# crockwell/far

Hardware: AMD Instinct MI355X
Metric: image-pairs/sec (match+solve+regress) at 640x480 (higher is better)
Workload: dtype f32

## Files before the change

far_amd/csrc/dual_softmax_f16s.hip:

```cpp
#include "k1_f16s.h"
#include <algorithm>

int far_k1_conf_launch(const _Float16* ah, const _Float16* bh, int Z, int L, int S, int Lp, int Sp, float c1, float fill2,
                       const uint8_t* mask0, const uint8_t* mask1, const float2* rowstat, const float* cmax,
                       const float* cinv, float* conf, const int* fix_count, const uint2* fix_list, int slots,
                       int* fix_info_out, hipStream_t stream);

namespace {

constexpr int CAND_SLOTS = 4;

#define FAR_DPP(old, v, ctrl, rowmask) \
    __builtin_bit_cast(float, __builtin_amdgcn_update_dpp(__builtin_bit_cast(int, old), __builtin_bit_cast(int, v), ctrl, rowmask, 0xF, false))
__device__ __forceinline__ float max32_to_upper_row(float v) {
    v = fmaxf(v, FAR_DPP(v, v, 0xB1, 0xF));
    v = fmaxf(v, FAR_DPP(v, v, 0x4E, 0xF));
    v = fmaxf(v, FAR_DPP(v, v, 0x141, 0xF));
    v = fmaxf(v, FAR_DPP(v, v, 0x140, 0xF));
    v = fmaxf(v, FAR_DPP(v, v, 0x142, 0xA));
    return v;
}

template <bool CAND>
__global__ __launch_bounds__(256, 2) void k1_rowstats(const _Float16* __restrict__ ah, const _Float16* __restrict__ al,
                                                      const _Float16* __restrict__ bh, const _Float16* __restrict__ bl,
                                                      int Z, int Nr, int Nc, int Nrp, int Ncp, float c1, float fill2,
                                                      const uint8_t* __restrict__ rmask, const uint8_t* __restrict__ cmask,
                                                      float2* __restrict__ stat, float* __restrict__ dmax, float* __restrict__ dinv,
                                                      float* __restrict__ dthr, const float* __restrict__ othr,
                                                      int* __restrict__ cand_count, uint2* __restrict__ cand) {
    extern __shared__ __attribute__((aligned(16))) unsigned char lds[];
    const int tid = threadIdx.x, wave = tid >> 6, lane = tid & 63, l31 = lane & 31, h = lane >> 5;
    int z, Ib;
    tile_coords(Nrp / 128, Z, z, Ib);
    const int irow = Ib * 128 + 32 * wave + l31;
    RowFrags rf;
    rf.load(ah, al, (size_t)z * Nrp + irow, irow, h);
    const bool rmasked = rmask && irow < Nr && !rmask[(size_t)z * Nr + irow];
    float m = -HUGE_F, sum = 0.f, comp = 0.f;
    int ncand = 0;
    const int ntile = (Nc + KT - 1) / KT;
    for (int jt = 0; jt < ntile; ++jt) {
        __syncthreads();
        dma_tile(lds, bh, bl, (size_t)z * Ncp + jt * KT, tid, wave);
        if (CAND && tid < KT)
            reinterpret_cast<float*>(lds + 2 * TILE_PLANE)[tid] = othr[(size_t)z * Ncp + jt * KT + tid];
        asm volatile("s_waitcnt vmcnt(0)" ::: "memory");
        __syncthreads();
        f32x16 acc[2];
        score_tile(acc, lds, rf, l31, h);
        const bool special = (jt + 1) * KT > Nc || cmask != nullptr || rmask != nullptr;
        float tm = -HUGE_F;
#pragma unroll
        for (int ct = 0; ct < 2; ++ct)
#pragma unroll
            for (int r = 0; r < 16; ++r) {
                float x = acc[ct][r] * c1;
                if (special) {
                    const int j = jt * KT + 32 * ct + mfma32_row(r, h);
                    if (j >= Nc) x = -HUGE_F;
                    else if (rmasked || (cmask && !cmask[(size_t)z * Nc + j])) x = fill2;
                }
                acc[ct][r] = x;
                tm = fmaxf(tm, x);
            }
        const float mn = fmaxf(m, tm);
        const float resc = __builtin_amdgcn_exp2f(m - mn);
        float t = 0.f;
#pragma unroll
        for (int ct = 0; ct < 2; ++ct)
#pragma unroll
            for (int r = 0; r < 16; ++r) t += __builtin_amdgcn_exp2f(acc[ct][r] - mn);
        sum *= resc;
        comp *= resc;
        const float y = t - comp;
        const float ns = sum + y;
        comp = (ns - sum) - y;
        sum = ns;
        m = mn;
        if (CAND) {
            const float clog = m + __builtin_amdgcn_logf(sum - comp);
            float hot = -1.f;
            const float* tl = reinterpret_cast<const float*>(lds + 2 * TILE_PLANE);
#pragma unroll
            for (int ct = 0; ct < 2; ++ct)
#pragma unroll
                for (int q4 = 0; q4 < 4; ++q4) {
                    const float4 a = *reinterpret_cast<const float4*>(tl + 32 * ct + 8 * q4 + 4 * h);
                    hot = fmaxf(hot, fmaxf(fmaxf(2.0f * acc[ct][4 * q4 + 0] - a.x, 2.0f * acc[ct][4 * q4 + 1] - a.y),
                                           fmaxf(2.0f * acc[ct][4 * q4 + 2] - a.z, 2.0f * acc[ct][4 * q4 + 3] - a.w)));
                }
            if (__builtin_amdgcn_ballot_w64(hot >= clog) != 0ull) {
                uint2* const slots = cand + ((size_t)z * Nr + min(irow, Nr - 1)) * (2 * CAND_SLOTS) + h * CAND_SLOTS;
#pragma unroll 1
                for (int ct = 0; ct < 2; ++ct)
#pragma unroll
                    for (int r = 0; r < 16; ++r) {
                        const int i = jt * KT + 32 * ct + mfma32_row(r, h);
                        const float xv = ct == 0 ? acc[0][r] : acc[1][r];
                        if (2.0f * xv >= tl[32 * ct + mfma32_row(r, h)] + clog && xv > -1.0e8f && i < Nc && irow < Nr) {
                            if (ncand < CAND_SLOTS) slots[ncand] = make_uint2((unsigned)i, __float_as_uint(xv));
                            ++ncand;
                        }
                    }
            }
        }
    }
    if (CAND && irow < Nr) cand_count[((size_t)z * Nr + irow) * 2 + h] = ncand;
    sum -= comp;
    const float mo = shfl_xor_f(m, 32), so = shfl_xor_f(sum, 32);
    const float mn = fmaxf(m, mo);
    const float st = sum * __builtin_amdgcn_exp2f(m - mn) + so * __builtin_amdgcn_exp2f(mo - mn);
    if (h == 0) {
        if (irow < Nr) stat[(size_t)z * Nr + irow] = make_float2(mn, st);
        if (dmax) {
            dmax[(size_t)z * Nrp + irow] = irow < Nr ? mn : HUGE_F;
            dinv[(size_t)z * Nrp + irow] = irow < Nr ? 1.0f / st : 0.f;
        }
        if (dthr) dthr[(size_t)z * Nrp + irow] = irow < Nr ? mn + __builtin_amdgcn_logf(st) - 12.0f : HUGE_F;
    }
}

__global__ __launch_bounds__(256, 2) void k1_screen(const _Float16* __restrict__ ah, const _Float16* __restrict__ bh, int Z, int L, int S,
                                                    int Lp, int Sp, float c1, const float2* __restrict__ rowstat,
                                                    const float* __restrict__ cmax, float thr, const unsigned* __restrict__ nmax,
                                                    uint8_t* __restrict__ tmask) {
    extern __shared__ __attribute__((aligned(16))) unsigned char lds[];
    const int tid = threadIdx.x, wave = tid >> 6, lane = tid & 63, l31 = lane & 31, h = lane >> 5;
    const int nI = Lp / 128;
    int z, Ib;
    tile_coords(nI, Z, z, Ib);
    const int irow = Ib * 128 + 32 * wave + l31;
    f16x8 rh[NS];
#pragma unroll
    for (int s = 0; s < NS; ++s)
        rh[s] = *reinterpret_cast<const f16x8*>(ah + ((size_t)z * Lp + irow) * C + 8 * ((2 * s + h) ^ (irow & 15)));
    const float rmax = irow < L ? rowstat[(size_t)z * L + irow].x : HUGE_F;
    const float c2 = 2.0f * c1;
    const float slack2 = c2 * __builtin_sqrtf(__uint_as_float(nmax[0]) * __uint_as_float(nmax[1])) *
                         (1.0f / 1024.0f * (1.0f + 1.0f / 2048.0f) + 1.0f / 8192.0f);
    const float lim = __builtin_amdgcn_logf(thr) + rmax - slack2;
    const int ntile = (S + KT - 1) / KT;
    for (int jt = 0; jt < ntile; ++jt) {
        __syncthreads();
        {
            const unsigned char* sh = reinterpret_cast<const unsigned char*>(bh + ((size_t)z * Sp + jt * KT) * C) + tid * 16;
#pragma unroll
            for (int j = 0; j < TILE_PLANE / 4096; ++j)
                __builtin_amdgcn_global_load_lds((gptr_t)(sh + j * 4096), (lptr_t)(lds + j * 4096 + wave * 1024), 16, 0, 0);
        }
        asm volatile("s_waitcnt vmcnt(0)" ::: "memory");
        __syncthreads();
        f32x16 acc[2];
#pragma unroll
        for (int ct = 0; ct < 2; ++ct)
#pragma unroll
            for (int r = 0; r < 16; ++r) acc[ct][r] = 0.f;
#pragma unroll
        for (int s = 0; s < NS; ++s)
#pragma unroll
            for (int ct = 0; ct < 2; ++ct) {
                const int row = 32 * ct + l31;
                const f16x8 ch = *reinterpret_cast<const f16x8*>(lds + row * ROWB + (((2 * s + h) ^ (row & 15)) * 16));
                acc[ct] = __builtin_amdgcn_mfma_f32_32x32x16_f16(ch, rh[s], acc[ct], 0, 0, 0);
            }
        float top = -HUGE_F;
#pragma unroll
        for (int ct = 0; ct < 2; ++ct)
#pragma unroll
            for (int q4 = 0; q4 < 4; ++q4) {
                const float4 a = *reinterpret_cast<const float4*>(cmax + (size_t)z * Sp + jt * KT + 32 * ct + 8 * q4 + 4 * h);
                top = fmaxf(top, fmaxf(fmaxf(fmaf(acc[ct][4 * q4 + 0], c2, -a.x), fmaf(acc[ct][4 * q4 + 1], c2, -a.y)),
                                       fmaxf(fmaf(acc[ct][4 * q4 + 2], c2, -a.z), fmaf(acc[ct][4 * q4 + 3], c2, -a.w))));
            }
        const bool can = !(top <= lim);
        const bool any = __builtin_amdgcn_ballot_w64(can) != 0ull;
        if (lane == 0) tmask[(((size_t)z * nI + Ib) * ntile + jt) * 4 + wave] = any ? 1 : 0;
    }
}

template <bool CONF>
__global__ __launch_bounds__(256, 2) void k1_match(const _Float16* __restrict__ ah, const _Float16* __restrict__ al,
                                                   const _Float16* __restrict__ bh, const _Float16* __restrict__ bl,
                                                   int Z, int L, int S, int Lp, int Sp, float c1, float fill2,
                                                   const uint8_t* __restrict__ mask0, const uint8_t* __restrict__ mask1,
                                                   const float2* __restrict__ rowstat, const float* __restrict__ cmax,
                                                   const float* __restrict__ cinv, float* __restrict__ conf,
                                                   float* __restrict__ rowbest_v, int* __restrict__ rowbest_j,
                                                   unsigned* __restrict__ colbest, float thr, const uint8_t* __restrict__ tmask) {
    extern __shared__ __attribute__((aligned(16))) unsigned char lds[];
    const int tid = threadIdx.x, wave = tid >> 6, lane = tid & 63, l31 = lane & 31, h = lane >> 5;
    const int nI = Lp / 128;
    int z, Ib;
    tile_coords(nI, Z, z, Ib);
    const int irow = Ib * 128 + 32 * wave + l31;
    const bool ivalid = irow < L;
    RowFrags rf;
    rf.load(ah, al, (size_t)z * Lp + irow, irow, h);
    const float2 rst = ivalid ? rowstat[(size_t)z * L + irow] : make_float2(0.f, 1.f);
    const float rinv = 1.0f / rst.y;
    const float c2 = 2.0f * c1;
    const bool rmasked = mask0 && ivalid && !mask0[(size_t)z * L + irow];
    const bool aligned4 = (S & 3) == 0;
    float bestv = -1.f;
    int bestj = 0x7fffffff;
    const int ntile = (S + KT - 1) / KT;
    for (int jt = 0; jt < ntile; ++jt) {
        if (tmask && *reinterpret_cast<const unsigned*>(tmask + (((size_t)z * nI + Ib) * ntile + jt) * 4) == 0u) continue;
        __syncthreads();
        dma_tile(lds, bh, bl, (size_t)z * Sp + jt * KT, tid, wave);
        asm volatile("s_waitcnt vmcnt(0)" ::: "memory");
        __syncthreads();
        if (tmask && tmask[(((size_t)z * nI + Ib) * ntile + jt) * 4 + wave] == 0) continue;
        f32x16 acc[2];
        score_tile(acc, lds, rf, l31, h);
        const bool masks = mask0 != nullptr || mask1 != nullptr;
#pragma unroll
        for (int ct = 0; ct < 2; ++ct) {
            float cm[16], ci[16];
#pragma unroll
            for (int q4 = 0; q4 < 4; ++q4) {
                const size_t o = (size_t)z * Sp + jt * KT + 32 * ct + 8 * q4 + 4 * h;
                const float4 a = *reinterpret_cast<const float4*>(cmax + o), b = *reinterpret_cast<const float4*>(cinv + o);
                cm[4 * q4 + 0] = a.x; cm[4 * q4 + 1] = a.y; cm[4 * q4 + 2] = a.z; cm[4 * q4 + 3] = a.w;
                ci[4 * q4 + 0] = b.x; ci[4 * q4 + 1] = b.y; ci[4 * q4 + 2] = b.z; ci[4 * q4 + 3] = b.w;
            }
#pragma unroll
            for (int r = 0; r < 16; ++r) {
                const int j = jt * KT + 32 * ct + mfma32_row(r, h);
                float x2 = acc[ct][r] * c2;
                if (masks && j < S && (rmasked || (mask1 && !mask1[(size_t)z * S + j]))) x2 = 2.0f * fill2;
                const float p = __builtin_amdgcn_exp2f((x2 - rst.x) - cm[r]) * rinv * ci[r];
                const bool valid = ivalid && j < S;
                acc[ct][r] = valid ? p : -1.f;
                if (valid && p > bestv) { bestv = p; bestj = j; }
            }
            if (CONF && ivalid) {
#pragma unroll
                for (int q4 = 0; q4 < 4; ++q4) {
                    const int j = jt * KT + 32 * ct + 8 * q4 + 4 * h;
                    float* dst = conf + ((size_t)z * L + irow) * S + j;
                    if (aligned4 && j + 3 < S) {
                        *reinterpret_cast<float4*>(dst) = make_float4(acc[ct][4 * q4], acc[ct][4 * q4 + 1], acc[ct][4 * q4 + 2], acc[ct][4 * q4 + 3]);
                    } else {
#pragma unroll
                        for (int e = 0; e < 4; ++e)
                            if (j + e < S) dst[e] = acc[ct][4 * q4 + e];
                    }
                }
            }
            float tmax = fmaxf(fmaxf(acc[ct][0], acc[ct][1]), fmaxf(acc[ct][2], acc[ct][3]));
#pragma unroll
            for (int r = 4; r < 16; r += 2) tmax = fmaxf(tmax, fmaxf(acc[ct][r], acc[ct][r + 1]));
            if (__builtin_amdgcn_ballot_w64(tmax > thr) != 0ull) {
#pragma unroll
                for (int r = 0; r < 16; ++r)
                    if (acc[ct][r] > thr)
                        atomicMax(colbest + (size_t)z * S + jt * KT + 32 * ct + mfma32_row(r, h), __float_as_uint(acc[ct][r]));
            }
        }
    }
    const float vo = shfl_xor_f(bestv, 32);
    const int jo = shfl_xor_i(bestj, 32);
    if (vo > bestv || (vo == bestv && jo < bestj)) { bestv = vo; bestj = jo; }
    if (h == 0 && ivalid) {
        rowbest_v[(size_t)z * L + irow] = bestv;
        rowbest_j[(size_t)z * L + irow] = bestj;
    }
}

struct Ws16 {
    K1Workspace k;
    _Float16 *ah, *al, *bh, *bl;
    float2* colstat2;
    float *cmax, *cinv;
    float* rthr;
    uint8_t* tmask;
    unsigned* nmax;
    int* fix_count;
    uint2* fix_list;
    size_t bytes;
};
inline Ws16 carve16(void* ws, int Z, int L, int S) {
    Ws16 w;
    w.k = carve(ws, Z, L, S);
    const int Lp = (L + 127) / 128 * 128, Sp = (S + 127) / 128 * 128;
    unsigned char* p = (unsigned char*)ws;
    size_t o = w.k.bytes;
    auto take = [&](size_t n) { unsigned char* r = p ? p + o : nullptr; o += align256(n); return r; };
    w.ah = (_Float16*)take((size_t)Z * Lp * C * 2); w.al = (_Float16*)take((size_t)Z * Lp * C * 2);
    w.bh = (_Float16*)take((size_t)Z * Sp * C * 2); w.bl = (_Float16*)take((size_t)Z * Sp * C * 2);
    w.colstat2 = (float2*)take((size_t)Z * S * 8);
    w.cmax = (float*)take((size_t)Z * Sp * 4); w.cinv = (float*)take((size_t)Z * Sp * 4);
    w.rthr = (float*)take((size_t)Z * Lp * 4);
    w.nmax = (unsigned*)take(2 * sizeof(unsigned));
    w.tmask = (uint8_t*)take((size_t)Z * (Lp / 128) * ((S + KT - 1) / KT) * 4);
    w.fix_count = (int*)take((size_t)Z * S * 2 * sizeof(int));
    w.fix_list = (uint2*)take((size_t)Z * S * 2 * CAND_SLOTS * sizeof(uint2));
    w.bytes = o;
    return w;
}

}

size_t far_k1_fwd_ws_bytes(int Z, int L, int S) { return carve16(nullptr, Z, L, S).bytes; }

static float k1_c1(float temperature) {
    return (float)(1.4426950408889634 / ((double)C * (double)temperature * PRESCALE * PRESCALE));
}

int far_k1_stats_launch_masked(const float* f0, const float* f1, int Z, int L, int S, float temperature, const uint8_t* mask0,
                               const uint8_t* mask1, void* ws, int* overflow, hipStream_t stream) {
    const Ws16 w = carve16(ws, Z, L, S);
    const int Lp = (L + 127) / 128 * 128, Sp = (S + 127) / 128 * 128;
    const float c1 = k1_c1(temperature), fill2 = -1e9f * 1.44269504088896341f;
    auto gridp = [](long n) { long b = (n + 255) / 256; return (unsigned)(b < 65536L * 4 ? b : 65536L * 4); };
    hipLaunchKernelGGL(k1_prep, dim3(gridp((long)Z * Lp * 32)), dim3(256), 0, stream, f0, Z, L, Lp, w.ah, w.al, overflow, (unsigned*)nullptr);
    hipLaunchKernelGGL(k1_prep, dim3(gridp((long)Z * Sp * 32)), dim3(256), 0, stream, f1, Z, S, Sp, w.bh, w.bl, overflow, (unsigned*)nullptr);
    const size_t smem_s = 2 * TILE_PLANE + KT * sizeof(float);
    FAR_ONCE_PER_DEVICE(hipFuncSetAttribute((const void*)k1_rowstats<false>, hipFuncAttributeMaxDynamicSharedMemorySize, (int)smem_s));
    hipLaunchKernelGGL(k1_rowstats<false>, dim3((Lp / 128) * Z), dim3(256), smem_s, stream, w.ah, w.al, w.bh, w.bl, Z, L, S, Lp, Sp,
                       c1, fill2, mask0, mask1, w.k.rowstat, (float*)nullptr, (float*)nullptr,
                       (float*)nullptr, (const float*)nullptr, (int*)nullptr, (uint2*)nullptr);
    hipLaunchKernelGGL(k1_rowstats<false>, dim3((Sp / 128) * Z), dim3(256), smem_s, stream, w.bh, w.bl, w.ah, w.al, Z, S, L, Sp, Lp,
                       c1, fill2, mask1, mask0, w.colstat2, w.cmax, w.cinv, (float*)nullptr,
                       (const float*)nullptr, (int*)nullptr, (uint2*)nullptr);
    return far_check_launch();
}

int far_k1_stats_launch(const float* f0, const float* f1, int Z, int L, int S, float temperature, void* ws, int* overflow,
                        hipStream_t stream) {
    return far_k1_stats_launch_masked(f0, f1, Z, L, S, temperature, nullptr, nullptr, ws, overflow, stream);
}

void far_k1_fwd_planes(void* ws, int Z, int L, int S, const _Float16** ah, const _Float16** al, const _Float16** bh,
                       const _Float16** bl, const float2** rowstat, const float2** colstat) {
    const Ws16 w = carve16(ws, Z, L, S);
    *ah = w.ah; *al = w.al; *bh = w.bh; *bl = w.bl; *rowstat = w.k.rowstat; *colstat = w.colstat2;
}

void far_k1_fwd_views(void* ws, int Z, int L, int S, const _Float16** ah, const _Float16** bh, const float2** rowstat,
                      const float** cmax, const float** cinv, float* c1_out) {
    const Ws16 w = carve16(ws, Z, L, S);
    *ah = w.ah; *bh = w.bh; *rowstat = w.k.rowstat; *cmax = w.cmax; *cinv = w.cinv;
    *c1_out = 0.f;
}

extern "C" {

size_t far_coarse_match_f16s_workspace_bytes(int Z, int L, int S, int Cc) {
    if (Z <= 0 || L <= 0 || S <= 0 || Cc != C) return 0;
    return carve16(nullptr, Z, L, S).bytes;
}

int far_coarse_match_f16s(const float* f0, const float* f1, int Z, int L, int S, int Cc,
                          float temperature, float thr, int border, int h0, int w0, int h1, int w1,
                          float cell_scale, const uint8_t* mask0, const uint8_t* mask1,
                          const int* valid_hw, const float* scale0, const float* scale1,
                          float* conf_out, int64_t* b_ids, int64_t* i_ids, int64_t* j_ids, float* mconf,
                          float* mkpts0_c, float* mkpts1_c, int* counts_out, int* total_out,
                          void* ws, int* overflow, hipStream_t stream) {
    far_clear_errors();
    if (!f0 || !f1 || !ws || !b_ids || !i_ids || !j_ids || !mconf || !mkpts0_c || !mkpts1_c || !total_out)
        return FAR_EINVAL;
    if (Z <= 0 || L <= 0 || S <= 0 || Cc != C || h0 * w0 != L || h1 * w1 != S || (long)Z * (L > S ? L : S) > 0x7ff00000L) return FAR_EINVAL;
    const Ws16 w = carve16(ws, Z, L, S);
    const int Lp = (L + 127) / 128 * 128, Sp = (S + 127) / 128 * 128;
    const float c1 = (float)(1.4426950408889634 / ((double)C * (double)temperature * PRESCALE * PRESCALE));
    const float fill2 = -1e9f * 1.44269504088896341f;
    auto gridp = [](long n) { long b = (n + 255) / 256; return (unsigned)(b < 65536L * 4 ? b : 65536L * 4); };
    const bool screen = !conf_out && !mask0 && !mask1 && far_get_tuning(10) == 0;
    if (screen) hipMemsetAsync(w.nmax, 0, 2 * sizeof(unsigned), stream);
    hipLaunchKernelGGL(k1_prep, dim3(gridp((long)Z * Lp * 32)), dim3(256), 0, stream, f0, Z, L, Lp, w.ah, w.al, overflow, screen ? w.nmax : (unsigned*)nullptr);
    hipLaunchKernelGGL(k1_prep, dim3(gridp((long)Z * Sp * 32)), dim3(256), 0, stream, f1, Z, S, Sp, w.bh, w.bl, overflow, screen ? w.nmax + 1 : (unsigned*)nullptr);
    int* counts = counts_out ? counts_out : w.k.counts;
    hipMemsetAsync(counts, 0, sizeof(int) * Z, stream);
    const size_t smem_s = 2 * TILE_PLANE + KT * sizeof(float), smem_m = 2 * TILE_PLANE + 4 * 64 * sizeof(float);
    FAR_ONCE_PER_DEVICE(
        hipFuncSetAttribute((const void*)k1_rowstats<false>, hipFuncAttributeMaxDynamicSharedMemorySize, (int)smem_s);
        hipFuncSetAttribute((const void*)k1_match<false>, hipFuncAttributeMaxDynamicSharedMemorySize, (int)smem_m);
        hipFuncSetAttribute((const void*)k1_match<true>, hipFuncAttributeMaxDynamicSharedMemorySize, (int)smem_m));
    hipLaunchKernelGGL(k1_rowstats<false>, dim3((Lp / 128) * Z), dim3(256), smem_s, stream, w.ah, w.al, w.bh, w.bl, Z, L, S, Lp, Sp,
                       c1, fill2, mask0, mask1, w.k.rowstat, (float*)nullptr, (float*)nullptr, (float*)nullptr,
                       (const float*)nullptr, (int*)nullptr, (uint2*)nullptr);
    hipLaunchKernelGGL(k1_rowstats<false>, dim3((Sp / 128) * Z), dim3(256), smem_s, stream, w.bh, w.bl, w.ah, w.al, Z, S, L, Sp, Lp,
                       c1, fill2, mask1, mask0, w.colstat2, w.cmax, w.cinv, (float*)nullptr, (const float*)nullptr,
                       (int*)nullptr, (uint2*)nullptr);
    const int nI = Lp / 128;
    hipMemsetAsync(w.k.colbest_part, 0, sizeof(float) * (size_t)Z * S, stream);
    if (screen) {
        FAR_ONCE_PER_DEVICE(hipFuncSetAttribute((const void*)k1_screen, hipFuncAttributeMaxDynamicSharedMemorySize, (int)TILE_PLANE));
        hipLaunchKernelGGL(k1_screen, dim3(nI * Z), dim3(256), TILE_PLANE, stream, w.ah, w.bh, Z, L, S, Lp, Sp, c1, w.k.rowstat, w.cmax, thr,
                           (const unsigned*)w.nmax, w.tmask);
    }
    if (conf_out)
        hipLaunchKernelGGL(k1_match<true>, dim3(nI * Z), dim3(256), smem_m, stream, w.ah, w.al, w.bh, w.bl, Z, L, S, Lp, Sp, c1,
                           fill2, mask0, mask1, w.k.rowstat, w.cmax, w.cinv, conf_out, w.k.rowbest_v, w.k.rowbest_j, reinterpret_cast<unsigned*>(w.k.colbest_part), thr,
                           screen ? (const uint8_t*)w.tmask : (const uint8_t*)nullptr);
    else
        hipLaunchKernelGGL(k1_match<false>, dim3(nI * Z), dim3(256), smem_m, stream, w.ah, w.al, w.bh, w.bl, Z, L, S, Lp, Sp, c1,
                           fill2, mask0, mask1, w.k.rowstat, w.cmax, w.cinv, conf_out, w.k.rowbest_v, w.k.rowbest_j, reinterpret_cast<unsigned*>(w.k.colbest_part), thr,
                           screen ? (const uint8_t*)w.tmask : (const uint8_t*)nullptr);
    hipLaunchKernelGGL(k_finalize, dim3((L + 255) / 256, Z), dim3(256), 0, stream, w.k.rowbest_v, w.k.rowbest_j,
                       w.k.colbest_part, 1, L, S, thr, border, h0, w0, h1, w1, valid_hw, w.k.match_j, counts);
    hipLaunchKernelGGL(k_compact, dim3(Z), dim3(256), 0, stream, w.k.match_j, w.k.rowbest_v, counts, L, w0, w1,
                       cell_scale, scale0, scale1, b_ids, i_ids, j_ids, mconf, mkpts0_c, mkpts1_c, total_out);
    return far_check_launch();
}

int far_conf_matrix_f16s(const float* f0, const float* f1, int Z, int L, int S, int Cc, float temperature,
                         const uint8_t* mask0, const uint8_t* mask1, int stages, float* conf_out, int* fix_info_out,
                         void* ws, int* overflow, hipStream_t stream) {
    far_clear_errors();
    if (!f0 || !f1 || !ws || !conf_out || Z <= 0 || L <= 0 || S <= 0 || Cc != C || !(stages & 3) || (long)Z * (L > S ? L : S) > 0x7ff00000L) return FAR_EINVAL;
    const Ws16 w = carve16(ws, Z, L, S);
    const int Lp = (L + 127) / 128 * 128, Sp = (S + 127) / 128 * 128;
    const float c1 = (float)(1.4426950408889634 / ((double)C * (double)temperature * PRESCALE * PRESCALE));
    const float fill2 = -1e9f * 1.44269504088896341f;
    if (stages & 1) {
        auto gridp = [](long n) { long b = (n + 255) / 256; return (unsigned)(b < 65536L * 4 ? b : 65536L * 4); };
        hipLaunchKernelGGL(k1_prep, dim3(gridp((long)Z * Lp * 32)), dim3(256), 0, stream, f0, Z, L, Lp, w.ah, w.al, overflow, (unsigned*)nullptr);
        hipLaunchKernelGGL(k1_prep, dim3(gridp((long)Z * Sp * 32)), dim3(256), 0, stream, f1, Z, S, Sp, w.bh, w.bl, overflow, (unsigned*)nullptr);
        const size_t smem_s = 2 * TILE_PLANE + KT * sizeof(float);
        FAR_ONCE_PER_DEVICE(
            hipFuncSetAttribute((const void*)k1_rowstats<false>, hipFuncAttributeMaxDynamicSharedMemorySize, (int)smem_s);
            hipFuncSetAttribute((const void*)k1_rowstats<true>, hipFuncAttributeMaxDynamicSharedMemorySize, (int)smem_s));
        hipLaunchKernelGGL(k1_rowstats<false>, dim3((Lp / 128) * Z), dim3(256), smem_s, stream, w.ah, w.al, w.bh, w.bl, Z, L, S, Lp,
                           Sp, c1, fill2, mask0, mask1, w.k.rowstat, (float*)nullptr, (float*)nullptr, w.rthr,
                           (const float*)nullptr, (int*)nullptr, (uint2*)nullptr);
        hipLaunchKernelGGL(k1_rowstats<true>, dim3((Sp / 128) * Z), dim3(256), smem_s, stream, w.bh, w.bl, w.ah, w.al, Z, S, L, Sp,
                           Lp, c1, fill2, mask1, mask0, w.colstat2, w.cmax, w.cinv, (float*)nullptr, (const float*)w.rthr,
                           w.fix_count, w.fix_list);
    }
    if (stages & 2) {
        const int rc = far_k1_conf_launch(w.ah, w.bh, Z, L, S, Lp, Sp, c1, fill2, mask0, mask1, w.k.rowstat, w.cmax, w.cinv,
                                          conf_out, w.fix_count, w.fix_list, CAND_SLOTS, fix_info_out, stream);
        if (rc != FAR_OK) return rc;
    }
    return far_check_launch();
}

}
```

far_amd/csrc/k1_f16s.h:

```cpp
#pragma once
#include "dual_softmax_common.h"

namespace {

using namespace far_ds;

typedef _Float16 f16x8 __attribute__((ext_vector_type(8)));
typedef __attribute__((address_space(1))) const void* gptr_t;
typedef __attribute__((address_space(3))) void* lptr_t;

constexpr int C = 256;
constexpr int NS = C / 16;
constexpr int KT = 64;
constexpr int ROWB = C * 2;
constexpr float PRESCALE = 16.0f;
constexpr float HUGE_F = 1.0e30f;
constexpr int TILE_PLANE = KT * ROWB;

__device__ __forceinline__ void split1(float x, _Float16& hi, _Float16& lo) {
    hi = (_Float16)x;
    lo = (_Float16)(x - (float)hi);
}

__global__ void k1_prep(const float* __restrict__ x, int Z, int N, int Np, _Float16* __restrict__ hi, _Float16* __restrict__ lo,
                        int* __restrict__ overflow, unsigned* __restrict__ nmax) {
    const long total = (long)Z * Np * 32;
    bool bad = false;
    float n2max = 0.f;
    for (long t = (long)blockIdx.x * blockDim.x + threadIdx.x; t < total; t += (long)gridDim.x * blockDim.x) {
        const int slot = (int)(t & 31);
        const long row = t >> 5;
        const unsigned urow = (unsigned)row, uz = urow / (unsigned)Np;
        const int i = (int)(urow - uz * (unsigned)Np);
        const long z = uz;
        f16x8 vh, vl;
        if (i < N) {
            const float* src = x + ((size_t)z * N + i) * C + slot * 8;
            const float4 a = *reinterpret_cast<const float4*>(src), b = *reinterpret_cast<const float4*>(src + 4);
            const float v[8] = {a.x, a.y, a.z, a.w, b.x, b.y, b.z, b.w};
#pragma unroll
            for (int e = 0; e < 8; ++e) {
                _Float16 h, l;
                split1(v[e] * PRESCALE, h, l);
                vh[e] = h; vl[e] = l;
                bad |= !(fabsf(v[e]) <= 65504.0f / PRESCALE);
            }
        } else {
#pragma unroll
            for (int e = 0; e < 8; ++e) { vh[e] = (_Float16)0.f; vl[e] = (_Float16)0.f; }
        }
        const int s2 = slot ^ (i & 15);
        *reinterpret_cast<f16x8*>(hi + (size_t)row * C + s2 * 8) = vh;
        *reinterpret_cast<f16x8*>(lo + (size_t)row * C + s2 * 8) = vl;
        if (nmax) {
            float n2 = 0.f;
#pragma unroll
            for (int e = 0; e < 8; ++e) { const float q = (float)vh[e] + (float)vl[e]; n2 = fmaf(q, q, n2); }
#pragma unroll
            for (int m = 1; m < 32; m <<= 1) n2 += shfl_xor_f(n2, m);
            n2max = fmaxf(n2max, n2);
        }
    }
    if (nmax) {
        n2max = fmaxf(n2max, shfl_xor_f(n2max, 32));
        if ((threadIdx.x & 63) == 0 && n2max > __uint_as_float(*reinterpret_cast<volatile unsigned*>(nmax))) atomicMax(nmax, __float_as_uint(n2max));
    }
    if (overflow && __any(bad) && (threadIdx.x & 63) == 0) atomicOr(overflow, 1);
}

struct RowFrags {
    f16x8 hi[NS], lo[NS];
    __device__ __forceinline__ void load(const _Float16* ph, const _Float16* pl, size_t row, int irow, int h) {
#pragma unroll
        for (int s = 0; s < NS; ++s) {
            const int slot = (2 * s + h) ^ (irow & 15);
            hi[s] = *reinterpret_cast<const f16x8*>(ph + row * C + 8 * slot);
            lo[s] = *reinterpret_cast<const f16x8*>(pl + row * C + 8 * slot);
        }
    }
};

__device__ __forceinline__ void dma_tile(unsigned char* lds, const _Float16* gh, const _Float16* gl, size_t row0, int tid, int wave) {
    const unsigned char* sh = reinterpret_cast<const unsigned char*>(gh + row0 * C) + tid * 16;
    const unsigned char* sl = reinterpret_cast<const unsigned char*>(gl + row0 * C) + tid * 16;
#pragma unroll
    for (int j = 0; j < TILE_PLANE / 4096; ++j) {
        __builtin_amdgcn_global_load_lds((gptr_t)(sh + j * 4096), (lptr_t)(lds + j * 4096 + wave * 1024), 16, 0, 0);
        __builtin_amdgcn_global_load_lds((gptr_t)(sl + j * 4096), (lptr_t)(lds + TILE_PLANE + j * 4096 + wave * 1024), 16, 0, 0);
    }
}

__device__ __forceinline__ void score_tile(f32x16 (&acc)[2], const unsigned char* lds, const RowFrags& rf, int l31, int h) {
#pragma unroll
    for (int ct = 0; ct < 2; ++ct)
#pragma unroll
        for (int r = 0; r < 16; ++r) acc[ct][r] = 0.f;
#pragma unroll
    for (int s = 0; s < NS; ++s) {
        f16x8 ch[2], cl[2];
#pragma unroll
        for (int ct = 0; ct < 2; ++ct) {
            const int row = 32 * ct + l31;
            const int off = row * ROWB + (((2 * s + h) ^ (row & 15)) * 16);
            ch[ct] = *reinterpret_cast<const f16x8*>(lds + off);
            cl[ct] = *reinterpret_cast<const f16x8*>(lds + TILE_PLANE + off);
        }
#pragma unroll
        for (int ct = 0; ct < 2; ++ct) acc[ct] = __builtin_amdgcn_mfma_f32_32x32x16_f16(ch[ct], rf.hi[s], acc[ct], 0, 0, 0);
#pragma unroll
        for (int ct = 0; ct < 2; ++ct) acc[ct] = __builtin_amdgcn_mfma_f32_32x32x16_f16(ch[ct], rf.lo[s], acc[ct], 0, 0, 0);
#pragma unroll
        for (int ct = 0; ct < 2; ++ct) acc[ct] = __builtin_amdgcn_mfma_f32_32x32x16_f16(cl[ct], rf.hi[s], acc[ct], 0, 0, 0);
    }
}

}

size_t far_k1_fwd_ws_bytes(int Z, int L, int S);
int far_k1_stats_launch(const float* f0, const float* f1, int Z, int L, int S, float temperature, void* ws, int* overflow,
                        hipStream_t stream);
int far_k1_stats_launch_masked(const float* f0, const float* f1, int Z, int L, int S, float temperature, const uint8_t* mask0,
                               const uint8_t* mask1, void* ws, int* overflow, hipStream_t stream);
void far_k1_fwd_views(void* ws, int Z, int L, int S, const _Float16** ah, const _Float16** bh, const float2** rowstat,
                      const float** cmax, const float** cinv, float* c1);
void far_k1_fwd_planes(void* ws, int Z, int L, int S, const _Float16** ah, const _Float16** al, const _Float16** bh,
                       const _Float16** bl, const float2** rowstat, const float2** colstat);

int far_skh_history_launch(const float* f0, const float* f1, int Z, int L, int S, const float* bin_score, int iters,
                           const uint8_t* mask0, const uint8_t* mask1, _Float16* ah, _Float16* al, _Float16* bh, _Float16* bl,
                           float* uh, float* vh, float* binh, int* overflow, hipStream_t stream);
```

far_amd/csrc/sinkhorn_f16s.hip:

```cpp
#include "k1_f16s.h"

namespace {

constexpr float LOG2E = 1.44269504088896341f;
constexpr float LN2 = 0.693147180559945309f;
constexpr float DEAD = -0.5f * HUGE_F;

__device__ __forceinline__ void lse_add(float& m, float& s, float v) {
    if (v > m) { s = s * __builtin_amdgcn_exp2f(m - v) + 1.0f; m = v; }
    else s += __builtin_amdgcn_exp2f(v - m);
}
__device__ __forceinline__ void lse_merge(float& m, float& s, float mo, float so) {
    const float mn = fmaxf(m, mo);
    s = s * __builtin_amdgcn_exp2f(m - mn) + so * __builtin_amdgcn_exp2f(mo - mn);
    m = mn;
}

__global__ void k_skh_init(float* __restrict__ up, int L, int Lp, float* __restrict__ vp, int S, int Sp, float* __restrict__ bins, int Z) {
    const long n = (long)Z * (Lp + Sp);
    for (long t = (long)blockIdx.x * blockDim.x + threadIdx.x; t < n; t += (long)gridDim.x * blockDim.x) {
        if (t < (long)Z * Lp) up[t] = (int)(t % Lp) < L ? 0.f : -HUGE_F;
        else { const long q = t - (long)Z * Lp; vp[q] = (int)(q % Sp) < S ? 0.f : -HUGE_F; }
    }
    if (blockIdx.x == 0)
        for (int t = threadIdx.x; t < 2 * Z; t += blockDim.x) bins[t] = 0.f;
}

template <bool FULL>
__global__ __launch_bounds__(256, 2) void k_skh_stats(const _Float16* __restrict__ ah, const _Float16* __restrict__ al,
                                                      const _Float16* __restrict__ bh, const _Float16* __restrict__ bl,
                                                      int Z, int Nr, int Nc, int Nrp, int Ncp, float c1,
                                                      const uint8_t* __restrict__ rmask, const uint8_t* __restrict__ cmask,
                                                      const float* __restrict__ cpot, const float* __restrict__ cbin,
                                                      const float* __restrict__ bin_score, float lmu, float lmu_bin,
                                                      float* __restrict__ rpot, float* __restrict__ rbin, float* __restrict__ rmax) {
    extern __shared__ __attribute__((aligned(16))) unsigned char lds[];
    const int tid = threadIdx.x, wave = tid >> 6, lane = tid & 63, l31 = lane & 31, h = lane >> 5;
    float* const tpot = reinterpret_cast<float*>(lds + 2 * TILE_PLANE);
    float* const red = tpot + KT;
    int z, Ib;
    tile_coords(Nrp / 128, Z, z, Ib);
    const float alpha = bin_score[0] * LOG2E;
    const float cb = cbin[z];
    if (FULL && Ib == 0) {
        float m = -HUGE_F, s = 0.f;
        for (int k = tid; k < Nc; k += 256) lse_add(m, s, cpot[(size_t)z * Ncp + k]);
#pragma unroll
        for (int o = 1; o < 64; o <<= 1) lse_merge(m, s, shfl_xor_f(m, o), shfl_xor_f(s, o));
        if (lane == 0) { red[2 * wave] = m; red[2 * wave + 1] = s; }
        __syncthreads();
        if (tid == 0) {
            float mm = red[0], ss = red[1];
            for (int w = 1; w < 4; ++w) lse_merge(mm, ss, red[2 * w], red[2 * w + 1]);
            lse_merge(mm, ss, cb, 1.0f);
            rbin[z] = lmu_bin - alpha - (mm + __builtin_amdgcn_logf(ss));
        }
    }
    const int irow = Ib * 128 + 32 * wave + l31;
    RowFrags rf;
    rf.load(ah, al, (size_t)z * Nrp + irow, irow, h);
    const bool rmasked = rmask && irow < Nr && !rmask[(size_t)z * Nr + irow];
    float m = -HUGE_F, sum = 0.f, comp = 0.f;
    const int ntile = (Nc + KT - 1) / KT;
    for (int jt = 0; jt < ntile; ++jt) {
        __syncthreads();
        dma_tile(lds, bh, bl, (size_t)z * Ncp + jt * KT, tid, wave);
        if (tid < KT) tpot[tid] = cpot[(size_t)z * Ncp + jt * KT + tid];
        asm volatile("s_waitcnt vmcnt(0)" ::: "memory");
        __syncthreads();
        f32x16 acc[2];
        score_tile(acc, lds, rf, l31, h);
        const bool special = (jt + 1) * KT > Nc || cmask != nullptr || rmask != nullptr;
        float tm = -HUGE_F;
#pragma unroll
        for (int ct = 0; ct < 2; ++ct)
#pragma unroll
            for (int q4 = 0; q4 < 4; ++q4) {
                const float4 pv = *reinterpret_cast<const float4*>(tpot + 32 * ct + 8 * q4 + 4 * h);
                const float p4[4] = {pv.x, pv.y, pv.z, pv.w};
#pragma unroll
                for (int e = 0; e < 4; ++e) {
                    const int r = 4 * q4 + e;
                    float x = fmaf(acc[ct][r], c1, p4[e]);
                    if (special) {
                        const int j = jt * KT + 32 * ct + mfma32_row(r, h);
                        if (j >= Nc || rmasked || (cmask && !cmask[(size_t)z * Nc + j])) x = -HUGE_F;
                    }
                    acc[ct][r] = x;
                    tm = fmaxf(tm, x);
                }
            }
        const float mn = fmaxf(m, tm);
        if (FULL) {
            const float resc = __builtin_amdgcn_exp2f(m - mn);
            float t = 0.f;
#pragma unroll
            for (int ct = 0; ct < 2; ++ct)
#pragma unroll
                for (int r = 0; r < 16; ++r) t += __builtin_amdgcn_exp2f(acc[ct][r] - mn);
            if (!(mn > DEAD)) t = 0.f;
            sum *= resc;
            comp *= resc;
            const float y = t - comp;
            const float ns = sum + y;
            comp = (ns - sum) - y;
            sum = ns;
        }
        m = mn;
    }
    const float mo = shfl_xor_f(m, 32);
    const float mn = fmaxf(m, mo);
    if (FULL) {
        sum -= comp;
        const float so = shfl_xor_f(sum, 32);
        float st = sum * __builtin_amdgcn_exp2f(m - mn) + so * __builtin_amdgcn_exp2f(mo - mn);
        float M = mn;
        lse_merge(M, st, alpha + cb, 1.0f);
        if (h == 0) rpot[(size_t)z * Nrp + irow] = irow < Nr ? lmu - (M + __builtin_amdgcn_logf(st)) : -HUGE_F;
    }
    if (rmax && h == 0) rmax[(size_t)z * Nrp + irow] = irow < Nr ? mn : -HUGE_F;
}

__global__ void k_skh_colfilter(const float* __restrict__ vp, const float* __restrict__ cmax, const float* __restrict__ ubin,
                                const float* __restrict__ bin_score, int Z, int S, int Sp, float* __restrict__ vm) {
    const long n = (long)Z * Sp;
    const float alpha = bin_score[0] * LOG2E;
    for (long t = (long)blockIdx.x * blockDim.x + threadIdx.x; t < n; t += (long)gridDim.x * blockDim.x) {
        const int z = (int)(t / Sp), j = (int)(t - (long)z * Sp);
        vm[t] = (j < S && !(alpha + ubin[z] > cmax[t])) ? vp[t] : -HUGE_F;
    }
}

template <bool CONF>
__global__ __launch_bounds__(256, 2) void k_skh_match(const _Float16* __restrict__ ah, const _Float16* __restrict__ al,
                                                      const _Float16* __restrict__ bh, const _Float16* __restrict__ bl,
                                                      int Z, int L, int S, int Lp, int Sp, float c1,
                                                      const uint8_t* __restrict__ mask0, const uint8_t* __restrict__ mask1,
                                                      const float* __restrict__ up, const float* __restrict__ vp,
                                                      const float* __restrict__ vbin, const float* __restrict__ rmax,
                                                      const float* __restrict__ bin_score, float nrm, float* __restrict__ conf,
                                                      float* __restrict__ rowbest_v, int* __restrict__ rowbest_j,
                                                      unsigned* __restrict__ colbest, float thr) {
    extern __shared__ __attribute__((aligned(16))) unsigned char lds[];
    const int tid = threadIdx.x, wave = tid >> 6, lane = tid & 63, l31 = lane & 31, h = lane >> 5;
    const int nI = Lp / 128;
    int z, Ib;
    tile_coords(nI, Z, z, Ib);
    const int irow = Ib * 128 + 32 * wave + l31;
    const bool ivalid = irow < L;
    RowFrags rf;
    rf.load(ah, al, (size_t)z * Lp + irow, irow, h);
    const float alpha = bin_score[0] * LOG2E;
    float un = up[(size_t)z * Lp + irow] - nrm;
    if (rmax && !(rmax[(size_t)z * Lp + irow] >= alpha + vbin[z])) un = -HUGE_F;
    const bool rmasked = mask0 && ivalid && !mask0[(size_t)z * L + irow];
    const bool masks = mask0 != nullptr || mask1 != nullptr;
    float bestv = -1.f;
    int bestj = 0x7fffffff;
    const int ntile = (S + KT - 1) / KT;
    for (int jt = 0; jt < ntile; ++jt) {
        __syncthreads();
        dma_tile(lds, bh, bl, (size_t)z * Sp + jt * KT, tid, wave);
        asm volatile("s_waitcnt vmcnt(0)" ::: "memory");
        __syncthreads();
        f32x16 acc[2];
        score_tile(acc, lds, rf, l31, h);
#pragma unroll
        for (int ct = 0; ct < 2; ++ct) {
#pragma unroll
            for (int q4 = 0; q4 < 4; ++q4) {
                const float4 pv = *reinterpret_cast<const float4*>(vp + (size_t)z * Sp + jt * KT + 32 * ct + 8 * q4 + 4 * h);
                const float p4[4] = {pv.x, pv.y, pv.z, pv.w};
#pragma unroll
                for (int e = 0; e < 4; ++e) {
                    const int r = 4 * q4 + e;
                    const int j = jt * KT + 32 * ct + mfma32_row(r, h);
                    float p = __builtin_amdgcn_exp2f(fmaf(acc[ct][r], c1, p4[e]) + un);
                    if (masks && j < S && (rmasked || (mask1 && !mask1[(size_t)z * S + j]))) p = 0.f;
                    const bool valid = ivalid && j < S;
                    acc[ct][r] = valid ? p : -1.f;
                    if (valid && p > bestv) { bestv = p; bestj = j; }
                }
            }
            if (CONF && ivalid) {
                float* dst = conf + ((size_t)z * (L + 1) + irow) * (S + 1);
#pragma unroll
                for (int r = 0; r < 16; ++r) {
                    const int j = jt * KT + 32 * ct + mfma32_row(r, h);
                    if (j < S) dst[j] = acc[ct][r];
                }
            }
            float tmax = fmaxf(fmaxf(acc[ct][0], acc[ct][1]), fmaxf(acc[ct][2], acc[ct][3]));
#pragma unroll
            for (int r = 4; r < 16; r += 2) tmax = fmaxf(tmax, fmaxf(acc[ct][r], acc[ct][r + 1]));
            if (__builtin_amdgcn_ballot_w64(tmax > thr) != 0ull) {
#pragma unroll
                for (int r = 0; r < 16; ++r)
                    if (acc[ct][r] > thr)
                        atomicMax(colbest + (size_t)z * S + jt * KT + 32 * ct + mfma32_row(r, h), __float_as_uint(acc[ct][r]));
            }
        }
    }
    const float vo = shfl_xor_f(bestv, 32);
    const int jo = shfl_xor_i(bestj, 32);
    if (vo > bestv || (vo == bestv && jo < bestj)) { bestv = vo; bestj = jo; }
    if (h == 0 && ivalid) {
        rowbest_v[(size_t)z * L + irow] = bestv;
        rowbest_j[(size_t)z * L + irow] = bestj;
    }
}

__global__ void k_skh_bins(const float* __restrict__ up, const float* __restrict__ vp, const float* __restrict__ bins,
                           const float* __restrict__ bin_score, int Z, int L, int S, int Lp, int Sp, float nrm,
                           float* __restrict__ conf, float* __restrict__ log_u, float* __restrict__ log_v) {
    const int z = blockIdx.y;
    const float alpha = bin_score[0] * LOG2E;
    const float ub = bins[z], vb = bins[Z + z];
    for (int t = blockIdx.x * blockDim.x + threadIdx.x; t < (L + 1) + (S + 1); t += gridDim.x * blockDim.x) {
        if (t <= L) {
            const float u = t < L ? up[(size_t)z * Lp + t] : ub;
            if (log_u) log_u[(size_t)z * (L + 1) + t] = u * LN2;
            if (conf) conf[((size_t)z * (L + 1) + t) * (S + 1) + S] = __builtin_amdgcn_exp2f(alpha + u + vb - nrm);
        } else {
            const int j = t - (L + 1);
            const float v = j < S ? vp[(size_t)z * Sp + j] : vb;
            if (log_v) log_v[(size_t)z * (S + 1) + j] = v * LN2;
            if (conf && j < S) conf[((size_t)z * (L + 1) + L) * (S + 1) + j] = __builtin_amdgcn_exp2f(alpha + ub + v - nrm);
        }
    }
}

struct WsSkh {
    _Float16 *ah, *al, *bh, *bl;
    float *up, *vp, *vm;
    float *rmax, *cmax;
    float* bins;
    float* rowbest_v; int* rowbest_j; unsigned* colbest; int* match_j; int* counts;
    size_t bytes;
};
inline WsSkh carve_skh(void* ws, int Z, int L, int S) {
    WsSkh w;
    const int Lp = (L + 127) / 128 * 128, Sp = (S + 127) / 128 * 128;
    unsigned char* p = (unsigned char*)ws;
    size_t o = 0;
    auto take = [&](size_t n) { unsigned char* r = p ? p + o : nullptr; o += align256(n); return r; };
    w.ah = (_Float16*)take((size_t)Z * Lp * C * 2); w.al = (_Float16*)take((size_t)Z * Lp * C * 2);
    w.bh = (_Float16*)take((size_t)Z * Sp * C * 2); w.bl = (_Float16*)take((size_t)Z * Sp * C * 2);
    w.up = (float*)take((size_t)Z * Lp * 4); w.vp = (float*)take((size_t)Z * Sp * 4); w.vm = (float*)take((size_t)Z * Sp * 4);
    w.rmax = (float*)take((size_t)Z * Lp * 4); w.cmax = (float*)take((size_t)Z * Sp * 4);
    w.bins = (float*)take((size_t)2 * Z * 4);
    w.rowbest_v = (float*)take((size_t)Z * L * 4); w.rowbest_j = (int*)take((size_t)Z * L * 4);
    w.colbest = (unsigned*)take((size_t)Z * S * 4); w.match_j = (int*)take((size_t)Z * L * 4);
    w.counts = (int*)take((size_t)(Z + 1) * 4);
    w.bytes = o;
    return w;
}

}

extern "C" {

size_t far_coarse_match_sinkhorn_f16s_workspace_bytes(int Z, int L, int S, int Cc) {
    if (Z <= 0 || L <= 0 || S <= 0 || Cc != C) return 0;
    return carve_skh(nullptr, Z, L, S).bytes;
}

int far_coarse_match_sinkhorn_f16s(const float* f0, const float* f1, int Z, int L, int S, int Cc,
                                   const float* bin_score, int iters, int prefilter, float thr, int border,
                                   int h0, int w0, int h1, int w1, float cell_scale, const uint8_t* mask0, const uint8_t* mask1,
                                   const int* valid_hw, const float* scale0, const float* scale1,
                                   float* conf_with_bin, float* log_u, float* log_v,
                                   int64_t* b_ids, int64_t* i_ids, int64_t* j_ids, float* mconf,
                                   float* mkpts0_c, float* mkpts1_c, int* counts_out, int* total_out,
                                   void* ws, int* overflow, hipStream_t stream) {
    far_clear_errors();
    if (!f0 || !f1 || !bin_score || !ws || !b_ids || !i_ids || !j_ids || !mconf || !mkpts0_c || !mkpts1_c || !total_out)
        return FAR_EINVAL;
    if (Z <= 0 || L <= 0 || S <= 0 || Cc != C || iters < 0 || h0 * w0 != L || h1 * w1 != S ||
        (long)Z * ((L > S ? L : S) + 128) > 0x7ff00000L)
        return FAR_EINVAL;
    const WsSkh w = carve_skh(ws, Z, L, S);
    const int Lp = (L + 127) / 128 * 128, Sp = (S + 127) / 128 * 128;
    const float c1 = (float)(1.4426950408889634 / ((double)C * PRESCALE * PRESCALE));
    const double n2 = -std::log2((double)L + (double)S);
    const float nrm = (float)n2, lmu_l = (float)(std::log2((double)S) + n2), lnu_s = (float)(std::log2((double)L) + n2);
    auto gridp = [](long n) { long b = (n + 255) / 256; return (unsigned)(b < 65536L * 4 ? b : 65536L * 4); };
    hipLaunchKernelGGL(k1_prep, dim3(gridp((long)Z * Lp * 32)), dim3(256), 0, stream, f0, Z, L, Lp, w.ah, w.al, overflow, (unsigned*)nullptr);
    hipLaunchKernelGGL(k1_prep, dim3(gridp((long)Z * Sp * 32)), dim3(256), 0, stream, f1, Z, S, Sp, w.bh, w.bl, overflow, (unsigned*)nullptr);
    hipLaunchKernelGGL(k_skh_init, dim3(gridp((long)Z * (Lp + Sp))), dim3(256), 0, stream, w.up, L, Lp, w.vp, S, Sp, w.bins, Z);
    int* counts = counts_out ? counts_out : w.counts;
    hipMemsetAsync(counts, 0, sizeof(int) * Z, stream);
    const size_t smem_s = 2 * TILE_PLANE + (KT + 8) * sizeof(float), smem_m = 2 * TILE_PLANE;
    FAR_ONCE_PER_DEVICE(
        hipFuncSetAttribute((const void*)k_skh_stats<true>, hipFuncAttributeMaxDynamicSharedMemorySize, (int)smem_s);
        hipFuncSetAttribute((const void*)k_skh_stats<false>, hipFuncAttributeMaxDynamicSharedMemorySize, (int)smem_s);
        hipFuncSetAttribute((const void*)k_skh_match<false>, hipFuncAttributeMaxDynamicSharedMemorySize, (int)smem_m);
        hipFuncSetAttribute((const void*)k_skh_match<true>, hipFuncAttributeMaxDynamicSharedMemorySize, (int)smem_m));
    float* const ubin = w.bins;
    float* const vbin = w.bins + Z;
    auto row_pass = [&](bool full, float* rmax) {
        hipLaunchKernelGGL(full ? k_skh_stats<true> : k_skh_stats<false>, dim3((Lp / 128) * Z), dim3(256), smem_s, stream,
                           w.ah, w.al, w.bh, w.bl, Z, L, S, Lp, Sp, c1, mask0, mask1, (const float*)w.vp, (const float*)vbin, bin_score,
                           nrm, lmu_l, w.up, ubin, rmax);
    };
    auto col_pass = [&](bool full, float* rmax) {
        hipLaunchKernelGGL(full ? k_skh_stats<true> : k_skh_stats<false>, dim3((Sp / 128) * Z), dim3(256), smem_s, stream,
                           w.bh, w.bl, w.ah, w.al, Z, S, L, Sp, Lp, c1, mask1, mask0, (const float*)w.up, (const float*)ubin, bin_score,
                           nrm, lnu_s, w.vp, vbin, rmax);
    };
    for (int t = 0; t < iters; ++t) {
        row_pass(true, nullptr);
        col_pass(true, prefilter && t == iters - 1 ? w.cmax : nullptr);
    }
    if (prefilter) {
        if (iters == 0) col_pass(false, w.cmax);
        row_pass(false, w.rmax);
        hipLaunchKernelGGL(k_skh_colfilter, dim3(gridp((long)Z * Sp)), dim3(256), 0, stream, (const float*)w.vp, (const float*)w.cmax,
                           (const float*)ubin, bin_score, Z, S, Sp, w.vm);
    }
    const float* vmatch = prefilter ? w.vm : w.vp;
    const float* rfilt = prefilter ? w.rmax : nullptr;
    const int nI = Lp / 128;
    hipMemsetAsync(w.colbest, 0, sizeof(unsigned) * (size_t)Z * S, stream);
    if (conf_with_bin)
        hipLaunchKernelGGL(k_skh_match<true>, dim3(nI * Z), dim3(256), smem_m, stream, w.ah, w.al, w.bh, w.bl, Z, L, S, Lp, Sp, c1,
                           mask0, mask1, (const float*)w.up, vmatch, (const float*)vbin, rfilt, bin_score, nrm, conf_with_bin,
                           w.rowbest_v, w.rowbest_j, w.colbest, thr);
    else
        hipLaunchKernelGGL(k_skh_match<false>, dim3(nI * Z), dim3(256), smem_m, stream, w.ah, w.al, w.bh, w.bl, Z, L, S, Lp, Sp, c1,
                           mask0, mask1, (const float*)w.up, vmatch, (const float*)vbin, rfilt, bin_score, nrm, conf_with_bin,
                           w.rowbest_v, w.rowbest_j, w.colbest, thr);
    if (conf_with_bin || log_u || log_v)
        hipLaunchKernelGGL(k_skh_bins, dim3((L + S + 2 + 255) / 256, Z), dim3(256), 0, stream, (const float*)w.up, (const float*)w.vp,
                           (const float*)w.bins, bin_score, Z, L, S, Lp, Sp, nrm, conf_with_bin, log_u, log_v);
    hipLaunchKernelGGL(k_finalize, dim3((L + 255) / 256, Z), dim3(256), 0, stream, w.rowbest_v, w.rowbest_j,
                       reinterpret_cast<const float*>(w.colbest), 1, L, S, thr, border, h0, w0, h1, w1, valid_hw, w.match_j, counts);
    hipLaunchKernelGGL(k_compact, dim3(Z), dim3(256), 0, stream, w.match_j, w.rowbest_v, counts, L, w0, w1,
                       cell_scale, scale0, scale1, b_ids, i_ids, j_ids, mconf, mkpts0_c, mkpts1_c, total_out);
    return far_check_launch();
}

}

int far_skh_history_launch(const float* f0, const float* f1, int Z, int L, int S, const float* bin_score, int iters,
                           const uint8_t* mask0, const uint8_t* mask1, _Float16* ah, _Float16* al, _Float16* bh, _Float16* bl,
                           float* uh, float* vh, float* binh, int* overflow, hipStream_t stream) {
    const int Lp = (L + 127) / 128 * 128, Sp = (S + 127) / 128 * 128;
    const float c1 = (float)(1.4426950408889634 / ((double)C * PRESCALE * PRESCALE));
    const double n2 = -std::log2((double)L + (double)S);
    const float nrm = (float)n2, lmu_l = (float)(std::log2((double)S) + n2), lnu_s = (float)(std::log2((double)L) + n2);
    auto gridp = [](long n) { long b = (n + 255) / 256; return (unsigned)(b < 65536L * 4 ? b : 65536L * 4); };
    hipLaunchKernelGGL(k1_prep, dim3(gridp((long)Z * Lp * 32)), dim3(256), 0, stream, f0, Z, L, Lp, ah, al, overflow, (unsigned*)nullptr);
    hipLaunchKernelGGL(k1_prep, dim3(gridp((long)Z * Sp * 32)), dim3(256), 0, stream, f1, Z, S, Sp, bh, bl, overflow, (unsigned*)nullptr);
    hipLaunchKernelGGL(k_skh_init, dim3(gridp((long)Z * (Lp + Sp))), dim3(256), 0, stream, uh, L, Lp, vh, S, Sp, binh, Z);
    const size_t smem_s = 2 * TILE_PLANE + (KT + 8) * sizeof(float);
    FAR_ONCE_PER_DEVICE(hipFuncSetAttribute((const void*)k_skh_stats<true>, hipFuncAttributeMaxDynamicSharedMemorySize, (int)smem_s));
    const size_t nu = (size_t)Z * Lp, nv = (size_t)Z * Sp;
    for (int t = 1; t <= iters; ++t) {
        float* const bt = binh + (size_t)t * 2 * Z;
        const float* const bp = binh + (size_t)(t - 1) * 2 * Z;
        hipLaunchKernelGGL(k_skh_stats<true>, dim3((Lp / 128) * Z), dim3(256), smem_s, stream, ah, al, bh, bl, Z, L, S, Lp, Sp, c1,
                           mask0, mask1, (const float*)(vh + (t - 1) * nv), bp + Z, bin_score, nrm, lmu_l, uh + t * nu, bt,
                           (float*)nullptr);
        hipLaunchKernelGGL(k_skh_stats<true>, dim3((Sp / 128) * Z), dim3(256), smem_s, stream, bh, bl, ah, al, Z, S, L, Sp, Lp, c1,
                           mask1, mask0, (const float*)(uh + t * nu), (const float*)bt, bin_score, nrm, lnu_s, vh + t * nv, bt + Z,
                           (float*)nullptr);
    }
    return far_check_launch();
}
```

Measured before the change: 376.4.

## Fold tile screening into column rowstats pass and double-buffer column tiles

Removes the separate k1_screen kernel. Tile-survival masks are now computed inside the column-side rowstats pass, using per-row thresholds written by the row pass, which drops the norm-max reduction from prep. The rowstats loop becomes a two-slot async global-to-LDS pipeline with scheduled MFMA/LDS interleaving, and prep plus the memsets are merged into one k1_prep_pair launch. The gains are one fewer GEMM-like pass, fewer launches and overlapped loads. The risk is that the new screening threshold and its slack differ from the old bound, which could change which tiles are kept.

```diff
diff --git a/far_amd/csrc/dual_softmax_f16s.hip b/far_amd/csrc/dual_softmax_f16s.hip
--- a/far_amd/csrc/dual_softmax_f16s.hip
+++ b/far_amd/csrc/dual_softmax_f16s.hip
@@ -21,34 +21,47 @@
     return v;
 }
 
-template <bool CAND>
+template <bool CAND, bool TILES = false>
 __global__ __launch_bounds__(256, 2) void k1_rowstats(const _Float16* __restrict__ ah, const _Float16* __restrict__ al,
                                                       const _Float16* __restrict__ bh, const _Float16* __restrict__ bl,
                                                       int Z, int Nr, int Nc, int Nrp, int Ncp, float c1, float fill2,
                                                       const uint8_t* __restrict__ rmask, const uint8_t* __restrict__ cmask,
                                                       float2* __restrict__ stat, float* __restrict__ dmax, float* __restrict__ dinv,
-                                                      float* __restrict__ dthr, const float* __restrict__ othr,
-                                                      int* __restrict__ cand_count, uint2* __restrict__ cand) {
+                                                      float* __restrict__ dthr, int dthr_tiles, float lt, const float* __restrict__ othr,
+                                                      int* __restrict__ cand_count, uint2* __restrict__ cand, uint8_t* __restrict__ tmask) {
     extern __shared__ __attribute__((aligned(16))) unsigned char lds[];
-    const int tid = threadIdx.x, wave = tid >> 6, lane = tid & 63, l31 = lane & 31, h = lane >> 5;
+    const int tid = threadIdx.x, wave = __builtin_amdgcn_readfirstlane(tid >> 6), lane = tid & 63, l31 = lane & 31, h = lane >> 5;
     int z, Ib;
     tile_coords(Nrp / 128, Z, z, Ib);
     const int irow = Ib * 128 + 32 * wave + l31;
     RowFrags rf;
     rf.load(ah, al, (size_t)z * Nrp + irow, irow, h);
     const bool rmasked = rmask && irow < Nr && !rmask[(size_t)z * Nr + irow];
+    rf.arrived();
     float m = -HUGE_F, sum = 0.f, comp = 0.f;
     int ncand = 0;
     const int ntile = (Nc + KT - 1) / KT;
+    unsigned char* const slot0 = lds;
+    unsigned char* const slot1 = lds + SLOT_BYTES;
+    float* const tbuf = reinterpret_cast<float*>(lds + 2 * SLOT_BYTES);
+    const size_t crow = (size_t)z * Ncp;
+    auto request0 = [&](int jt) {
+        dma_slot_async(slot0, bh, bl, crow + jt * KT, tid, wave);
+        if ((CAND || TILES) && wave == 0)
+            glds4(othr + crow + jt * KT + lane, lds_addr_uniform(reinterpret_cast<const unsigned char*>(tbuf + (jt & 1) * KT)));
+    };
+    request0(0);
     for (int jt = 0; jt < ntile; ++jt) {
-        __syncthreads();
-        dma_tile(lds, bh, bl, (size_t)z * Ncp + jt * KT, tid, wave);
-        if (CAND && tid < KT)
-            reinterpret_cast<float*>(lds + 2 * TILE_PLANE)[tid] = othr[(size_t)z * Ncp + jt * KT + tid];
-        asm volatile("s_waitcnt vmcnt(0)" ::: "memory");
-        __syncthreads();
         f32x16 acc[2];
-        score_tile(acc, lds, rf, l31, h);
+        ring_wait();
+        ring_barrier();
+        dma_slot_async(slot1, bh, bl, crow + jt * KT + SLOT_COLS, tid, wave);
+        score_slot(acc[0], slot0, rf, l31, h);
+        ring_wait();
+        ring_barrier();
+        if (jt + 1 < ntile) request0(jt + 1);
+        score_slot(acc[1], slot1, rf, l31, h);
+        const float* const tl = tbuf + (jt & 1) * KT;
         const bool special = (jt + 1) * KT > Nc || cmask != nullptr || rmask != nullptr;
         float tm = -HUGE_F;
 #pragma unroll
@@ -81,7 +94,6 @@
         if (CAND) {
             const float clog = m + __builtin_amdgcn_logf(sum - comp);
             float hot = -1.f;
-            const float* tl = reinterpret_cast<const float*>(lds + 2 * TILE_PLANE);
 #pragma unroll
             for (int ct = 0; ct < 2; ++ct)
 #pragma unroll
@@ -103,6 +115,21 @@
                             ++ncand;
                         }
                     }
+            }
+        }
+        if (TILES) {
+            const int jtile = Ib * 2 + (wave >> 1), nI = Ncp / 128, njt = (Nr + KT - 1) / KT;
+#pragma unroll
+            for (int ct = 0; ct < 2; ++ct) {
+                float hot = -HUGE_F;
+#pragma unroll
+                for (int q4 = 0; q4 < 4; ++q4) {
+                    const float4 a = *reinterpret_cast<const float4*>(tl + 32 * ct + 8 * q4 + 4 * h);
+                    hot = fmaxf(hot, fmaxf(fmaxf(2.0f * acc[ct][4 * q4 + 0] - a.x, 2.0f * acc[ct][4 * q4 + 1] - a.y),
+                                           fmaxf(2.0f * acc[ct][4 * q4 + 2] - a.z, 2.0f * acc[ct][4 * q4 + 3] - a.w)));
+                }
+                const bool any = __builtin_amdgcn_ballot_w64(!(hot <= m)) != 0ull;
+                if (any && lane == 0 && jtile < njt) tmask[(((size_t)z * nI + (jt >> 1)) * njt + jtile) * 4 + (jt & 1) * 2 + ct] = 1;
             }
         }
     }
@@ -117,65 +144,10 @@
             dmax[(size_t)z * Nrp + irow] = irow < Nr ? mn : HUGE_F;
             dinv[(size_t)z * Nrp + irow] = irow < Nr ? 1.0f / st : 0.f;
         }
-        if (dthr) dthr[(size_t)z * Nrp + irow] = irow < Nr ? mn + __builtin_amdgcn_logf(st) - 12.0f : HUGE_F;
-    }
-}
-
-__global__ __launch_bounds__(256, 2) void k1_screen(const _Float16* __restrict__ ah, const _Float16* __restrict__ bh, int Z, int L, int S,
-                                                    int Lp, int Sp, float c1, const float2* __restrict__ rowstat,
-                                                    const float* __restrict__ cmax, float thr, const unsigned* __restrict__ nmax,
-                                                    uint8_t* __restrict__ tmask) {
-    extern __shared__ __attribute__((aligned(16))) unsigned char lds[];
-    const int tid = threadIdx.x, wave = tid >> 6, lane = tid & 63, l31 = lane & 31, h = lane >> 5;
-    const int nI = Lp / 128;
-    int z, Ib;
-    tile_coords(nI, Z, z, Ib);
-    const int irow = Ib * 128 + 32 * wave + l31;
-    f16x8 rh[NS];
-#pragma unroll
-    for (int s = 0; s < NS; ++s)
-        rh[s] = *reinterpret_cast<const f16x8*>(ah + ((size_t)z * Lp + irow) * C + 8 * ((2 * s + h) ^ (irow & 15)));
-    const float rmax = irow < L ? rowstat[(size_t)z * L + irow].x : HUGE_F;
-    const float c2 = 2.0f * c1;
-    const float slack2 = c2 * __builtin_sqrtf(__uint_as_float(nmax[0]) * __uint_as_float(nmax[1])) *
-                         (1.0f / 1024.0f * (1.0f + 1.0f / 2048.0f) + 1.0f / 8192.0f);
-    const float lim = __builtin_amdgcn_logf(thr) + rmax - slack2;
-    const int ntile = (S + KT - 1) / KT;
-    for (int jt = 0; jt < ntile; ++jt) {
-        __syncthreads();
-        {
-            const unsigned char* sh = reinterpret_cast<const unsigned char*>(bh + ((size_t)z * Sp + jt * KT) * C) + tid * 16;
-#pragma unroll
-            for (int j = 0; j < TILE_PLANE / 4096; ++j)
-                __builtin_amdgcn_global_load_lds((gptr_t)(sh + j * 4096), (lptr_t)(lds + j * 4096 + wave * 1024), 16, 0, 0);
-        }
-        asm volatile("s_waitcnt vmcnt(0)" ::: "memory");
-        __syncthreads();
-        f32x16 acc[2];
-#pragma unroll
-        for (int ct = 0; ct < 2; ++ct)
-#pragma unroll
-            for (int r = 0; r < 16; ++r) acc[ct][r] = 0.f;
-#pragma unroll
-        for (int s = 0; s < NS; ++s)
-#pragma unroll
-            for (int ct = 0; ct < 2; ++ct) {
-                const int row = 32 * ct + l31;
-                const f16x8 ch = *reinterpret_cast<const f16x8*>(lds + row * ROWB + (((2 * s + h) ^ (row & 15)) * 16));
-                acc[ct] = __builtin_amdgcn_mfma_f32_32x32x16_f16(ch, rh[s], acc[ct], 0, 0, 0);
-            }
-        float top = -HUGE_F;
-#pragma unroll
-        for (int ct = 0; ct < 2; ++ct)
-#pragma unroll
-            for (int q4 = 0; q4 < 4; ++q4) {
-                const float4 a = *reinterpret_cast<const float4*>(cmax + (size_t)z * Sp + jt * KT + 32 * ct + 8 * q4 + 4 * h);
-                top = fmaxf(top, fmaxf(fmaxf(fmaf(acc[ct][4 * q4 + 0], c2, -a.x), fmaf(acc[ct][4 * q4 + 1], c2, -a.y)),
-                                       fmaxf(fmaf(acc[ct][4 * q4 + 2], c2, -a.z), fmaf(acc[ct][4 * q4 + 3], c2, -a.w))));
-            }
-        const bool can = !(top <= lim);
-        const bool any = __builtin_amdgcn_ballot_w64(can) != 0ull;
-        if (lane == 0) tmask[(((size_t)z * nI + Ib) * ntile + jt) * 4 + wave] = any ? 1 : 0;
+        if (dthr)
+            dthr[(size_t)z * Nrp + irow] = irow >= Nr ? HUGE_F
+                                           : dthr_tiles ? mn + lt - (1.0f / 1024.0f + fabsf(mn) * (1.0f / 524288.0f))
+                                                        : mn + __builtin_amdgcn_logf(st) - 12.0f;
     }
 }
 
@@ -276,7 +248,6 @@
     float *cmax, *cinv;
     float* rthr;
     uint8_t* tmask;
-    unsigned* nmax;
     int* fix_count;
     uint2* fix_list;
     size_t bytes;
@@ -293,12 +264,36 @@
     w.colstat2 = (float2*)take((size_t)Z * S * 8);
     w.cmax = (float*)take((size_t)Z * Sp * 4); w.cinv = (float*)take((size_t)Z * Sp * 4);
     w.rthr = (float*)take((size_t)Z * Lp * 4);
-    w.nmax = (unsigned*)take(2 * sizeof(unsigned));
+    take(2 * sizeof(unsigned));
     w.tmask = (uint8_t*)take((size_t)Z * (Lp / 128) * ((S + KT - 1) / KT) * 4);
     w.fix_count = (int*)take((size_t)Z * S * 2 * sizeof(int));
     w.fix_list = (uint2*)take((size_t)Z * S * 2 * CAND_SLOTS * sizeof(uint2));
     w.bytes = o;
     return w;
+}
+
+template <bool CAND, bool TILES>
+void launch_rowstats(hipStream_t stream, const _Float16* ah, const _Float16* al, const _Float16* bh, const _Float16* bl, int Z, int Nr,
+                     int Nc, int Nrp, int Ncp, float c1, float fill2, const uint8_t* rmask, const uint8_t* cmask, float2* stat,
+                     float* dmax, float* dinv, float* dthr, int dthr_tiles, float lt, const float* othr, int* cand_count, uint2* cand,
+                     uint8_t* tmask) {
+    const size_t smem = 2 * SLOT_BYTES + 2 * KT * sizeof(float);
+    FAR_ONCE_PER_DEVICE(hipFuncSetAttribute((const void*)k1_rowstats<CAND, TILES>, hipFuncAttributeMaxDynamicSharedMemorySize, (int)smem));
+    hipLaunchKernelGGL((k1_rowstats<CAND, TILES>), dim3((Nrp / 128) * Z), dim3(256), smem, stream, ah, al, bh, bl, Z, Nr, Nc, Nrp, Ncp, c1,
+                       fill2, rmask, cmask, stat, dmax, dinv, dthr, dthr_tiles, lt, othr, cand_count, cand, tmask);
+}
+
+__global__ void k1_prep_pair(const float* __restrict__ f0, const float* __restrict__ f1, int Z, int L, int S, int Lp, int Sp,
+                             _Float16* __restrict__ ah, _Float16* __restrict__ al, _Float16* __restrict__ bh, _Float16* __restrict__ bl,
+                             int* __restrict__ overflow, int* __restrict__ counts, unsigned* __restrict__ colbest, long ncol,
+                             unsigned* __restrict__ tmask4, long ntm) {
+    const long t0 = (long)blockIdx.x * blockDim.x + threadIdx.x, stride = (long)gridDim.x * blockDim.x;
+    bool bad = prep_slots(f0, Z, L, Lp, ah, al, t0, stride);
+    bad |= prep_slots(f1, Z, S, Sp, bh, bl, t0, stride);
+    for (long t = t0; t < Z; t += stride) counts[t] = 0;
+    for (long t = t0; t < ncol; t += stride) colbest[t] = 0u;
+    for (long t = t0; t < ntm; t += stride) tmask4[t] = 0u;
+    if (overflow && __any(bad) && (threadIdx.x & 63) == 0) atomicOr(overflow, 1);
 }
 
 }
@@ -315,16 +310,12 @@
     const int Lp = (L + 127) / 128 * 128, Sp = (S + 127) / 128 * 128;
     const float c1 = k1_c1(temperature), fill2 = -1e9f * 1.44269504088896341f;
     auto gridp = [](long n) { long b = (n + 255) / 256; return (unsigned)(b < 65536L * 4 ? b : 65536L * 4); };
-    hipLaunchKernelGGL(k1_prep, dim3(gridp((long)Z * Lp * 32)), dim3(256), 0, stream, f0, Z, L, Lp, w.ah, w.al, overflow, (unsigned*)nullptr);
-    hipLaunchKernelGGL(k1_prep, dim3(gridp((long)Z * Sp * 32)), dim3(256), 0, stream, f1, Z, S, Sp, w.bh, w.bl, overflow, (unsigned*)nullptr);
-    const size_t smem_s = 2 * TILE_PLANE + KT * sizeof(float);
-    FAR_ONCE_PER_DEVICE(hipFuncSetAttribute((const void*)k1_rowstats<false>, hipFuncAttributeMaxDynamicSharedMemorySize, (int)smem_s));
-    hipLaunchKernelGGL(k1_rowstats<false>, dim3((Lp / 128) * Z), dim3(256), smem_s, stream, w.ah, w.al, w.bh, w.bl, Z, L, S, Lp, Sp,
-                       c1, fill2, mask0, mask1, w.k.rowstat, (float*)nullptr, (float*)nullptr,
-                       (float*)nullptr, (const float*)nullptr, (int*)nullptr, (uint2*)nullptr);
-    hipLaunchKernelGGL(k1_rowstats<false>, dim3((Sp / 128) * Z), dim3(256), smem_s, stream, w.bh, w.bl, w.ah, w.al, Z, S, L, Sp, Lp,
-                       c1, fill2, mask1, mask0, w.colstat2, w.cmax, w.cinv, (float*)nullptr,
-                       (const float*)nullptr, (int*)nullptr, (uint2*)nullptr);
+    hipLaunchKernelGGL(k1_prep, dim3(gridp((long)Z * Lp * 32)), dim3(256), 0, stream, f0, Z, L, Lp, w.ah, w.al, overflow);
+    hipLaunchKernelGGL(k1_prep, dim3(gridp((long)Z * Sp * 32)), dim3(256), 0, stream, f1, Z, S, Sp, w.bh, w.bl, overflow);
+    launch_rowstats<false, false>(stream, w.ah, w.al, w.bh, w.bl, Z, L, S, Lp, Sp, c1, fill2, mask0, mask1, w.k.rowstat, nullptr, nullptr,
+                                  nullptr, 0, 0.f, nullptr, nullptr, nullptr, nullptr);
+    launch_rowstats<false, false>(stream, w.bh, w.bl, w.ah, w.al, Z, S, L, Sp, Lp, c1, fill2, mask1, mask0, w.colstat2, w.cmax, w.cinv,
+                                  nullptr, 0, 0.f, nullptr, nullptr, nullptr, nullptr);
     return far_check_launch();
 }
 
@@ -370,29 +361,24 @@
     const float fill2 = -1e9f * 1.44269504088896341f;
     auto gridp = [](long n) { long b = (n + 255) / 256; return (unsigned)(b < 65536L * 4 ? b : 65536L * 4); };
     const bool screen = !conf_out && !mask0 && !mask1 && far_get_tuning(10) == 0;
-    if (screen) hipMemsetAsync(w.nmax, 0, 2 * sizeof(unsigned), stream);
-    hipLaunchKernelGGL(k1_prep, dim3(gridp((long)Z * Lp * 32)), dim3(256), 0, stream, f0, Z, L, Lp, w.ah, w.al, overflow, screen ? w.nmax : (unsigned*)nullptr);
-    hipLaunchKernelGGL(k1_prep, dim3(gridp((long)Z * Sp * 32)), dim3(256), 0, stream, f1, Z, S, Sp, w.bh, w.bl, overflow, screen ? w.nmax + 1 : (unsigned*)nullptr);
     int* counts = counts_out ? counts_out : w.k.counts;
-    hipMemsetAsync(counts, 0, sizeof(int) * Z, stream);
-    const size_t smem_s = 2 * TILE_PLANE + KT * sizeof(float), smem_m = 2 * TILE_PLANE + 4 * 64 * sizeof(float);
+    const int nI = Lp / 128;
+    hipLaunchKernelGGL(k1_prep_pair, dim3(gridp((long)Z * (Lp > Sp ? Lp : Sp) * 32)), dim3(256), 0, stream, f0, f1, Z, L, S, Lp, Sp, w.ah, w.al,
+                       w.bh, w.bl, overflow, counts, reinterpret_cast<unsigned*>(w.k.colbest_part), (long)Z * S,
+                       reinterpret_cast<unsigned*>(w.tmask), screen ? (long)Z * nI * ((S + KT - 1) / KT) : 0L);
+    const size_t smem_m = 2 * TILE_PLANE + 4 * 64 * sizeof(float);
     FAR_ONCE_PER_DEVICE(
-        hipFuncSetAttribute((const void*)k1_rowstats<false>, hipFuncAttributeMaxDynamicSharedMemorySize, (int)smem_s);
         hipFuncSetAttribute((const void*)k1_match<false>, hipFuncAttributeMaxDynamicSharedMemorySize, (int)smem_m);
         hipFuncSetAttribute((const void*)k1_match<true>, hipFuncAttributeMaxDynamicSharedMemorySize, (int)smem_m));
-    hipLaunchKernelGGL(k1_rowstats<false>, dim3((Lp / 128) * Z), dim3(256), smem_s, stream, w.ah, w.al, w.bh, w.bl, Z, L, S, Lp, Sp,
-                       c1, fill2, mask0, mask1, w.k.rowstat, (float*)nullptr, (float*)nullptr, (float*)nullptr,
-                       (const float*)nullptr, (int*)nullptr, (uint2*)nullptr);
-    hipLaunchKernelGGL(k1_rowstats<false>, dim3((Sp / 128) * Z), dim3(256), smem_s, stream, w.bh, w.bl, w.ah, w.al, Z, S, L, Sp, Lp,
-                       c1, fill2, mask1, mask0, w.colstat2, w.cmax, w.cinv, (float*)nullptr, (const float*)nullptr,
-                       (int*)nullptr, (uint2*)nullptr);
-    const int nI = Lp / 128;
-    hipMemsetAsync(w.k.colbest_part, 0, sizeof(float) * (size_t)Z * S, stream);
-    if (screen) {
-        FAR_ONCE_PER_DEVICE(hipFuncSetAttribute((const void*)k1_screen, hipFuncAttributeMaxDynamicSharedMemorySize, (int)TILE_PLANE));
-        hipLaunchKernelGGL(k1_screen, dim3(nI * Z), dim3(256), TILE_PLANE, stream, w.ah, w.bh, Z, L, S, Lp, Sp, c1, w.k.rowstat, w.cmax, thr,
-                           (const unsigned*)w.nmax, w.tmask);
-    }
+    const float lt = thr > 0.f ? log2f(thr) : -INFINITY;
+    launch_rowstats<false, false>(stream, w.ah, w.al, w.bh, w.bl, Z, L, S, Lp, Sp, c1, fill2, mask0, mask1, w.k.rowstat, nullptr, nullptr,
+                                  screen ? w.rthr : nullptr, 1, lt, nullptr, nullptr, nullptr, nullptr);
+    if (screen)
+        launch_rowstats<false, true>(stream, w.bh, w.bl, w.ah, w.al, Z, S, L, Sp, Lp, c1, fill2, mask1, mask0, w.colstat2, w.cmax, w.cinv,
+                                     nullptr, 0, 0.f, w.rthr, nullptr, nullptr, w.tmask);
+    else
+        launch_rowstats<false, false>(stream, w.bh, w.bl, w.ah, w.al, Z, S, L, Sp, Lp, c1, fill2, mask1, mask0, w.colstat2, w.cmax, w.cinv,
+                                      nullptr, 0, 0.f, nullptr, nullptr, nullptr, nullptr);
     if (conf_out)
         hipLaunchKernelGGL(k1_match<true>, dim3(nI * Z), dim3(256), smem_m, stream, w.ah, w.al, w.bh, w.bl, Z, L, S, Lp, Sp, c1,
                            fill2, mask0, mask1, w.k.rowstat, w.cmax, w.cinv, conf_out, w.k.rowbest_v, w.k.rowbest_j, reinterpret_cast<unsigned*>(w.k.colbest_part), thr,
@@ -419,18 +405,12 @@
     const float fill2 = -1e9f * 1.44269504088896341f;
     if (stages & 1) {
         auto gridp = [](long n) { long b = (n + 255) / 256; return (unsigned)(b < 65536L * 4 ? b : 65536L * 4); };
-        hipLaunchKernelGGL(k1_prep, dim3(gridp((long)Z * Lp * 32)), dim3(256), 0, stream, f0, Z, L, Lp, w.ah, w.al, overflow, (unsigned*)nullptr);
-        hipLaunchKernelGGL(k1_prep, dim3(gridp((long)Z * Sp * 32)), dim3(256), 0, stream, f1, Z, S, Sp, w.bh, w.bl, overflow, (unsigned*)nullptr);
-        const size_t smem_s = 2 * TILE_PLANE + KT * sizeof(float);
-        FAR_ONCE_PER_DEVICE(
-            hipFuncSetAttribute((const void*)k1_rowstats<false>, hipFuncAttributeMaxDynamicSharedMemorySize, (int)smem_s);
-            hipFuncSetAttribute((const void*)k1_rowstats<true>, hipFuncAttributeMaxDynamicSharedMemorySize, (int)smem_s));
-        hipLaunchKernelGGL(k1_rowstats<false>, dim3((Lp / 128) * Z), dim3(256), smem_s, stream, w.ah, w.al, w.bh, w.bl, Z, L, S, Lp,
-                           Sp, c1, fill2, mask0, mask1, w.k.rowstat, (float*)nullptr, (float*)nullptr, w.rthr,
-                           (const float*)nullptr, (int*)nullptr, (uint2*)nullptr);
-        hipLaunchKernelGGL(k1_rowstats<true>, dim3((Sp / 128) * Z), dim3(256), smem_s, stream, w.bh, w.bl, w.ah, w.al, Z, S, L, Sp,
-                           Lp, c1, fill2, mask1, mask0, w.colstat2, w.cmax, w.cinv, (float*)nullptr, (const float*)w.rthr,
-                           w.fix_count, w.fix_list);
+        hipLaunchKernelGGL(k1_prep, dim3(gridp((long)Z * Lp * 32)), dim3(256), 0, stream, f0, Z, L, Lp, w.ah, w.al, overflow);
+        hipLaunchKernelGGL(k1_prep, dim3(gridp((long)Z * Sp * 32)), dim3(256), 0, stream, f1, Z, S, Sp, w.bh, w.bl, overflow);
+        launch_rowstats<false, false>(stream, w.ah, w.al, w.bh, w.bl, Z, L, S, Lp, Sp, c1, fill2, mask0, mask1, w.k.rowstat, nullptr, nullptr,
+                                      w.rthr, 0, 0.f, nullptr, nullptr, nullptr, nullptr);
+        launch_rowstats<true, false>(stream, w.bh, w.bl, w.ah, w.al, Z, S, L, Sp, Lp, c1, fill2, mask1, mask0, w.colstat2, w.cmax, w.cinv,
+                                     nullptr, 0, 0.f, w.rthr, w.fix_count, w.fix_list, nullptr);
     }
     if (stages & 2) {
         const int rc = far_k1_conf_launch(w.ah, w.bh, Z, L, S, Lp, Sp, c1, fill2, mask0, mask1, w.k.rowstat, w.cmax, w.cinv,
diff --git a/far_amd/csrc/k1_f16s.h b/far_amd/csrc/k1_f16s.h
--- a/far_amd/csrc/k1_f16s.h
+++ b/far_amd/csrc/k1_f16s.h
@@ -22,12 +22,11 @@
     lo = (_Float16)(x - (float)hi);
 }
 
-__global__ void k1_prep(const float* __restrict__ x, int Z, int N, int Np, _Float16* __restrict__ hi, _Float16* __restrict__ lo,
-                        int* __restrict__ overflow, unsigned* __restrict__ nmax) {
+__device__ __forceinline__ bool prep_slots(const float* __restrict__ x, int Z, int N, int Np, _Float16* __restrict__ hi,
+                                           _Float16* __restrict__ lo, long t0, long stride) {
     const long total = (long)Z * Np * 32;
     bool bad = false;
-    float n2max = 0.f;
-    for (long t = (long)blockIdx.x * blockDim.x + threadIdx.x; t < total; t += (long)gridDim.x * blockDim.x) {
+    for (long t = t0; t < total; t += stride) {
         const int slot = (int)(t & 31);
         const long row = t >> 5;
         const unsigned urow = (unsigned)row, uz = urow / (unsigned)Np;
@@ -52,19 +51,13 @@
         const int s2 = slot ^ (i & 15);
         *reinterpret_cast<f16x8*>(hi + (size_t)row * C + s2 * 8) = vh;
         *reinterpret_cast<f16x8*>(lo + (size_t)row * C + s2 * 8) = vl;
-        if (nmax) {
-            float n2 = 0.f;
-#pragma unroll
-            for (int e = 0; e < 8; ++e) { const float q = (float)vh[e] + (float)vl[e]; n2 = fmaf(q, q, n2); }
-#pragma unroll
-            for (int m = 1; m < 32; m <<= 1) n2 += shfl_xor_f(n2, m);
-            n2max = fmaxf(n2max, n2);
-        }
     }
-    if (nmax) {
-        n2max = fmaxf(n2max, shfl_xor_f(n2max, 32));
-        if ((threadIdx.x & 63) == 0 && n2max > __uint_as_float(*reinterpret_cast<volatile unsigned*>(nmax))) atomicMax(nmax, __float_as_uint(n2max));
-    }
+    return bad;
+}
+
+__global__ void k1_prep(const float* __restrict__ x, int Z, int N, int Np, _Float16* __restrict__ hi, _Float16* __restrict__ lo,
+                        int* __restrict__ overflow) {
+    const bool bad = prep_slots(x, Z, N, Np, hi, lo, (long)blockIdx.x * blockDim.x + threadIdx.x, (long)gridDim.x * blockDim.x);
     if (overflow && __any(bad) && (threadIdx.x & 63) == 0) atomicOr(overflow, 1);
 }
 
@@ -76,6 +69,15 @@
             const int slot = (2 * s + h) ^ (irow & 15);
             hi[s] = *reinterpret_cast<const f16x8*>(ph + row * C + 8 * slot);
             lo[s] = *reinterpret_cast<const f16x8*>(pl + row * C + 8 * slot);
+        }
+    }
+    __device__ __forceinline__ void arrived() {
+#pragma unroll
+        for (int s = 0; s < NS; s += 8) {
+            asm volatile("s_waitcnt vmcnt(0)" : "+v"(hi[s]), "+v"(hi[s + 1]), "+v"(hi[s + 2]), "+v"(hi[s + 3]),
+                                                "+v"(hi[s + 4]), "+v"(hi[s + 5]), "+v"(hi[s + 6]), "+v"(hi[s + 7]) : : "memory");
+            asm volatile("s_waitcnt vmcnt(0)" : "+v"(lo[s]), "+v"(lo[s + 1]), "+v"(lo[s + 2]), "+v"(lo[s + 3]),
+                                                "+v"(lo[s + 4]), "+v"(lo[s + 5]), "+v"(lo[s + 6]), "+v"(lo[s + 7]) : : "memory");
         }
     }
 };
@@ -114,6 +116,64 @@
     }
 }
 
+constexpr int SLOT_COLS = 32;
+constexpr int SLOT_PLANE = SLOT_COLS * ROWB;
+constexpr int SLOT_BYTES = 2 * SLOT_PLANE;
+__device__ __forceinline__ void glds16(const void* gsrc, unsigned lds_dst_uniform) {
+    unsigned keep;
+    asm volatile("s_mov_b32 %0, m0\n\ts_mov_b32 m0, %2\n\ts_nop 0\n\tglobal_load_lds_dwordx4 %1, off\n\ts_mov_b32 m0, %0"
+                 : "=&s"(keep) : "v"(gsrc), "s"(lds_dst_uniform) : "memory");
+}
+__device__ __forceinline__ void glds4(const void* gsrc, unsigned lds_dst_uniform) {
+    unsigned keep;
+    asm volatile("s_mov_b32 %0, m0\n\ts_mov_b32 m0, %2\n\ts_nop 0\n\tglobal_load_lds_dword %1, off\n\ts_mov_b32 m0, %0"
+                 : "=&s"(keep) : "v"(gsrc), "s"(lds_dst_uniform) : "memory");
+}
+__device__ __forceinline__ unsigned lds_addr_uniform(const unsigned char* p) {
+    return (unsigned)__builtin_amdgcn_readfirstlane((int)(unsigned)(size_t)(lptr_t)p);
+}
+__device__ __forceinline__ void ring_wait() { asm volatile("s_waitcnt vmcnt(0)" ::: "memory"); }
+
+__device__ __forceinline__ void dma_slot_async(unsigned char* slot, const _Float16* gh, const _Float16* gl, size_t row0, int tid, int wave) {
+    const unsigned char* sh = reinterpret_cast<const unsigned char*>(gh + row0 * C) + tid * 16;
+    const unsigned char* sl = reinterpret_cast<const unsigned char*>(gl + row0 * C) + tid * 16;
+    const unsigned dst = lds_addr_uniform(slot + wave * 1024);
+#pragma unroll
+    for (int j = 0; j < SLOT_PLANE / 4096; ++j) {
+        glds16(sh + j * 4096, dst + j * 4096);
+        glds16(sl + j * 4096, dst + SLOT_PLANE + j * 4096);
+    }
+}
+
+__device__ __forceinline__ void score_slot(f32x16& acc, const unsigned char* slot, const RowFrags& rf, int l31, int h) {
+#pragma unroll
+    for (int r = 0; r < 16; ++r) acc[r] = 0.f;
+    const unsigned char* const base = slot + l31 * ROWB;
+    const int key = l31 & 15;
+    f16x8 ch = *reinterpret_cast<const f16x8*>(base + ((h ^ key) * 16));
+    f16x8 cl = *reinterpret_cast<const f16x8*>(base + SLOT_PLANE + ((h ^ key) * 16));
+#pragma unroll
+    for (int s = 0; s < NS; ++s) {
+        f16x8 nh = ch, nl = cl;
+        if (s + 1 < NS) {
+            const int off = ((2 * (s + 1) + h) ^ key) * 16;
+            nh = *reinterpret_cast<const f16x8*>(base + off);
+            nl = *reinterpret_cast<const f16x8*>(base + SLOT_PLANE + off);
+        }
+        acc = __builtin_amdgcn_mfma_f32_32x32x16_f16(ch, rf.hi[s], acc, 0, 0, 0);
+        acc = __builtin_amdgcn_mfma_f32_32x32x16_f16(ch, rf.lo[s], acc, 0, 0, 0);
+        acc = __builtin_amdgcn_mfma_f32_32x32x16_f16(cl, rf.hi[s], acc, 0, 0, 0);
+        ch = nh; cl = nl;
+    }
+    __builtin_amdgcn_sched_group_barrier(0x100, 2, 0);
+#pragma unroll
+    for (int s = 0; s + 1 < NS; ++s) {
+        __builtin_amdgcn_sched_group_barrier(0x100, 2, 0);
+        __builtin_amdgcn_sched_group_barrier(0x008, 3, 0);
+    }
+    __builtin_amdgcn_sched_group_barrier(0x008, 3, 0);
+}
+
 }
 
 size_t far_k1_fwd_ws_bytes(int Z, int L, int S);
diff --git a/far_amd/csrc/sinkhorn_f16s.hip b/far_amd/csrc/sinkhorn_f16s.hip
--- a/far_amd/csrc/sinkhorn_f16s.hip
+++ b/far_amd/csrc/sinkhorn_f16s.hip
@@ -285,8 +285,8 @@
     const double n2 = -std::log2((double)L + (double)S);
     const float nrm = (float)n2, lmu_l = (float)(std::log2((double)S) + n2), lnu_s = (float)(std::log2((double)L) + n2);
     auto gridp = [](long n) { long b = (n + 255) / 256; return (unsigned)(b < 65536L * 4 ? b : 65536L * 4); };
-    hipLaunchKernelGGL(k1_prep, dim3(gridp((long)Z * Lp * 32)), dim3(256), 0, stream, f0, Z, L, Lp, w.ah, w.al, overflow, (unsigned*)nullptr);
-    hipLaunchKernelGGL(k1_prep, dim3(gridp((long)Z * Sp * 32)), dim3(256), 0, stream, f1, Z, S, Sp, w.bh, w.bl, overflow, (unsigned*)nullptr);
+    hipLaunchKernelGGL(k1_prep, dim3(gridp((long)Z * Lp * 32)), dim3(256), 0, stream, f0, Z, L, Lp, w.ah, w.al, overflow);
+    hipLaunchKernelGGL(k1_prep, dim3(gridp((long)Z * Sp * 32)), dim3(256), 0, stream, f1, Z, S, Sp, w.bh, w.bl, overflow);
     hipLaunchKernelGGL(k_skh_init, dim3(gridp((long)Z * (Lp + Sp))), dim3(256), 0, stream, w.up, L, Lp, w.vp, S, Sp, w.bins, Z);
     int* counts = counts_out ? counts_out : w.counts;
     hipMemsetAsync(counts, 0, sizeof(int) * Z, stream);
@@ -350,8 +350,8 @@
     const double n2 = -std::log2((double)L + (double)S);
     const float nrm = (float)n2, lmu_l = (float)(std::log2((double)S) + n2), lnu_s = (float)(std::log2((double)L) + n2);
     auto gridp = [](long n) { long b = (n + 255) / 256; return (unsigned)(b < 65536L * 4 ? b : 65536L * 4); };
-    hipLaunchKernelGGL(k1_prep, dim3(gridp((long)Z * Lp * 32)), dim3(256), 0, stream, f0, Z, L, Lp, ah, al, overflow, (unsigned*)nullptr);
-    hipLaunchKernelGGL(k1_prep, dim3(gridp((long)Z * Sp * 32)), dim3(256), 0, stream, f1, Z, S, Sp, bh, bl, overflow, (unsigned*)nullptr);
+    hipLaunchKernelGGL(k1_prep, dim3(gridp((long)Z * Lp * 32)), dim3(256), 0, stream, f0, Z, L, Lp, ah, al, overflow);
+    hipLaunchKernelGGL(k1_prep, dim3(gridp((long)Z * Sp * 32)), dim3(256), 0, stream, f1, Z, S, Sp, bh, bl, overflow);
     hipLaunchKernelGGL(k_skh_init, dim3(gridp((long)Z * (Lp + Sp))), dim3(256), 0, stream, uh, L, Lp, vh, S, Sp, binh, Z);
     const size_t smem_s = 2 * TILE_PLANE + (KT + 8) * sizeof(float);
     FAR_ONCE_PER_DEVICE(hipFuncSetAttribute((const void*)k_skh_stats<true>, hipFuncAttributeMaxDynamicSharedMemorySize, (int)smem_s));
```

New measurement: 378.5, median of 6. Within noise of the previous version (+0.6%).
